# rajgandhi1/threecrate

Measured on AMD Instinct MI355X. Metric: ICP iterations/sec (whole job: k=16 normals + 50-iter point-to-plane ICP per 1M-pt pair; tc_cloud handles, inputs resident in HBM), higher is better.
Workload: dtype f32; 1 GPU; 1000000-pt uniform-random cloud, k=16 normals + 50-iter point-to-plane ICP, independent sigma = 0.0001 noise on source and target, correspondences returned (BASELINE configs[1]; one independent pair per GPU); points=1000000, k=16, parallelism=pairs1, interface=tc_cloud handles (one index build per cloud)

## Files before the change

threecrate_amd/csrc/icp.hip:

```cpp
#include "tc_internal.h"
#include <hip/hip_ext.h>

#include <algorithm>
#include <type_traits>
#include <cmath>
#include <cstring>
#include <cstdlib>
#include <cstdio>

namespace tc {

typedef uint32_t u32x16 __attribute__((ext_vector_type(16)));
struct IcpHeader {
    float q[4], t[3];
    float prev_mse, conv_thr, max_dist;
    uint32_t iterations;
    int32_t done;
    float d_ang, d_t;
    uint32_t d_run;
};
static_assert(offsetof(IcpState, done) == 48 && offsetof(IcpState, max_dist) == 60 && offsetof(IcpState, iterations) == 36 &&
              offsetof(IcpState, prev_mse) == 28 && offsetof(IcpState, conv_thr) == 56, "IcpState header layout");
__device__ __forceinline__ IcpHeader load_header(const IcpState *st) {
    const u32x16 h = *reinterpret_cast<const u32x16 *>(st);
// ... 96 lines not shown
constexpr int kSpanRows = 9;

typedef uint32_t u32x4 __attribute__((ext_vector_type(4)));
typedef uint32_t u32x3 __attribute__((ext_vector_type(3)));

typedef float f32x4 __attribute__((ext_vector_type(4)));
typedef float f32x2 __attribute__((ext_vector_type(2)));

__device__ __forceinline__ float d2_packed(const f32x3 &c, const f32x2 &qxy, float qz) {
    const f32x2 dxy = c.xy - qxy;
    const float dz = c.z - qz;
    const f32x2 sxy = dxy * dxy;
    return (sxy.x + sxy.y) + dz * dz;
}

#ifdef TC_PHASE_STAMPS
#define TC_STAMP(i) do { const unsigned long long t_ = __builtin_amdgcn_s_memtime(); ph[i] += t_ - tl; tl = t_; } while (0)
#define TC_STAMP_ARGS , unsigned long long (&ph)[8], unsigned long long &tl
#define TC_STAMP_PASS , ph, tl
#else
#define TC_STAMP(i) do { } while (0)
#define TC_STAMP_ARGS
#define TC_STAMP_PASS
#endif
template <bool STATS = false, bool T2 = false>
__device__ __forceinline__ void nn_search_pruned(const GridView &gv, float x, float y, float z, float ub2,
                                                 float &best, uint32_t &bestj, bool &refine, float max_dist,
                                                 uint2 (*spans)[kIcpBlock], uint32_t &nsteps, const float *pts12, bool track2, float &low2 TC_STAMP_ARGS
                                                 ) {
    const GridGeom &g = gv.g;
    int cx, cy, cz;
    float out2;
    const float qx = fminf(fmaxf(x, g.minx), g.maxx), qy = fminf(fmaxf(y, g.miny), g.maxy),
                qz = fminf(fmaxf(z, g.minz), g.maxz);
    cx = cell_coord(qx, g.minx, g.inv_h, g.gx);
    cy = cell_coord(qy, g.miny, g.inv_h, g.gy);
    cz = cell_coord(qz, g.minz, g.inv_h, g.gz);
    const float fx = (qx - g.minx) * g.inv_h - (float)cx, fy = (qy - g.miny) * g.inv_h - (float)cy,
                fz = (qz - g.minz) * g.inv_h - (float)cz;
    out2 = outside_d2(x, y, z, qx, qy, qz, g.clamped);
    const float lo_x = fmaxf(fx - 2e-3f, 0.0f) * g.h, hi_x = fmaxf(1.0f - fx - 2e-3f, 0.0f) * g.h;
    const float lo_y = fmaxf(fy - 2e-3f, 0.0f) * g.h, hi_y = fmaxf(1.0f - fy - 2e-3f, 0.0f) * g.h;
    const float lo_z = fmaxf(fz - 2e-3f, 0.0f) * g.h, hi_z = fmaxf(1.0f - fz - 2e-3f, 0.0f) * g.h;
    const float ax2[3] = {lo_x * lo_x, 0.0f, hi_x * hi_x};
    const float ay2[3] = {lo_y * lo_y, 0.0f, hi_y * hi_y};
    const float az2[3] = {lo_z * lo_z, 0.0f, hi_z * hi_z};
// ... 484 lines not shown
#pragma unroll
            for (int w2 = 0; w2 < kIcpBlock / 64; ++w2) sum += red[w2][threadIdx.x];
        }
        partials[(size_t)blockIdx.x * TC_ICP_SUMS_STRIDE + threadIdx.x] = sum;
    }
    if (lane == 0) rlist[blockIdx.x * kWavesPerBlock + w] = wcnt;
    if (blk_times && threadIdx.x == 0) {
        blk_times[2 * blockIdx.x] = t_begin;
        blk_times[2 * blockIdx.x + 1] = __builtin_amdgcn_s_memrealtime();
#ifdef TC_PHASE_STAMPS
        TC_STAMP(6);
        for (int i = 0; i < 8; ++i) blk_times[2 * kMaxPartialBlocks + 8 * blockIdx.x + i] = ph[i];
#endif
    }
}

constexpr int kRefineThreads = 1024;
#ifndef TC_REFINE_LANES
#define TC_REFINE_LANES 32
#endif
constexpr int kRG = TC_REFINE_LANES;
constexpr int kRB = 4;

__device__ __forceinline__ unsigned long long group_min_u64(unsigned long long v) {
#pragma unroll
    for (int o = kRG / 2; o > 0; o >>= 1) {
        const unsigned long long w = __shfl_xor(v, o);
        v = w < v ? w : v;
    }
    return v;
}

__device__ __forceinline__ void shell_cell(int idx, int R, int W, int V, int &ox, int &oy, int &oz) {
    const int nz = 2 * W * W, ny = 2 * W * V;
    if (idx < nz) {
        const int f = idx / (W * W), r = idx - f * W * W;
        oz = f ? R : -R; oy = r / W - R; ox = r - (r / W) * W - R;
    } else if (idx < nz + ny) {
        const int i2 = idx - nz, f = i2 / (W * V), r = i2 - f * W * V;
        oy = f ? R : -R; oz = r / W - (R - 1); ox = r - (r / W) * W - R;
    } else {
        const int i3 = idx - nz - ny, f = i3 / (V * V), r = i3 - f * V * V;
        ox = f ? R : -R; oz = r / V - (R - 1); oy = r - (r / V) * V - (R - 1);
    }
}

// ... 113 lines not shown
                const unsigned long long kc = ka < kb ? ka : kb;
                lk = kc < lk ? kc : lk;
            }
        }
        lim = fminf(lim, __uint_as_float((uint32_t)(lk >> 32)));
        if ((batch & 3u) == 3u) {
            float gl = lim;
#pragma unroll
            for (int o = kRG / 2; o > 0; o >>= 1) gl = fminf(gl, __shfl_xor(gl, o));
            lim = gl;
        }
    }
    return group_min_u64(lk);
}

template <int MODE>
__global__ void __launch_bounds__(kRefineThreads) icp_refine_kernel(
    GridView tgt, const float4 *__restrict__ tgt_nrm, const float4 *__restrict__ src,
    IcpState *__restrict__ st, uint32_t *__restrict__ corr_pos , uint32_t *__restrict__ rlist,
    const double *__restrict__ main_rows, uint32_t n_main_rows, uint32_t seg_stride, double *__restrict__ partial_rows,
    const float4 *__restrict__ src_cov, int dbg) {
    constexpr bool P2PLANE = MODE == 1;
    constexpr int NACC = MODE == 0 ? TC_ICP_SUMS_P2P : TC_ICP_SUMS_P2PLANE;
    const IcpHeader hd = load_header(st);
    const bool dbg_shells = (dbg & 8192) != 0;
    __shared__ float lacc[kRefineThreads / kRG][TC_ICP_SUMS_STRIDE];
    const uint32_t rows_per = (n_main_rows + gridDim.x - 1) / gridDim.x;
    const uint32_t mr0 = min(blockIdx.x * rows_per, n_main_rows), mr1 = min(mr0 + rows_per, n_main_rows);
    constexpr int kFoldBatch = kMaxPartialBlocks / kRefineBlocks;
    double fr[kFoldBatch];
#pragma unroll
    for (int k = 0; k < kFoldBatch; ++k) {
        const double v = main_rows[(size_t)min(mr0 + k, n_main_rows - 1) * TC_ICP_SUMS_STRIDE + (threadIdx.x & (TC_ICP_SUMS_STRIDE - 1))];
        fr[k] = (mr0 + k < mr1) ? v : 0.0;
    }
    constexpr int kSegPerRow = kIcpBlock / 64;
    constexpr int kCntPer = kMaxPartialBlocks * kSegPerRow / kRefineThreads;
    const uint32_t n_segs = n_main_rows * kSegPerRow;
    constexpr uint32_t per = kCntPer;
    uint32_t cnt[kCntPer];
#pragma unroll
    for (int k = 0; k < kCntPer; ++k) {
        const uint32_t b = threadIdx.x * per + k;
        const uint32_t v = rlist[min(b, n_segs - 1)];
        cnt[k] = b < n_segs ? v : 0u;
    }
    if (hd.done) return;
    double folded = 0.0;
#pragma unroll
    for (int k = 0; k < kFoldBatch; ++k) folded += fr[k];
    if (threadIdx.x < TC_ICP_SUMS_STRIDE)
        for (uint32_t r = mr0 + kFoldBatch; r < mr1; ++r) folded += main_rows[(size_t)r * TC_ICP_SUMS_STRIDE + threadIdx.x];
    const GridGeom &g = tgt.g;
    const float q[4] = {hd.q[0], hd.q[1], hd.q[2], hd.q[3]};
    const float max_dist = hd.max_dist;
    __shared__ uint32_t seg_off[kMaxPartialBlocks * kSegPerRow + 1];
    __shared__ uint32_t wave_tot[kRefineThreads / 64];
    {
        uint32_t run = 0;
#pragma unroll
        for (int k = 0; k < kCntPer; ++k) run += cnt[k];
        uint32_t inc = run;
#pragma unroll
        for (int o = 1; o < 64; o <<= 1) {
            const uint32_t v = __shfl_up(inc, o);
            if ((int)(threadIdx.x & 63) >= o) inc += v;
        }
        if ((threadIdx.x & 63) == 63) wave_tot[threadIdx.x >> 6] = inc;
        __syncthreads();
        uint32_t ex = inc - run;
        for (int w2 = 0; w2 < (int)(threadIdx.x >> 6); ++w2) ex += wave_tot[w2];
#pragma unroll
        for (int k = 0; k < kCntPer; ++k) {
            const uint32_t b = threadIdx.x * per + k;
            if (b <= n_segs) seg_off[b] = ex;
            ex += cnt[k];
        }
        if (threadIdx.x == kRefineThreads - 1) seg_off[n_segs] = ex;
        __syncthreads();
    }
    const uint32_t count = seg_off[n_segs];
    const uint4 *__restrict__ entries = refine_entries(rlist);
    if (blockIdx.x == 0 && threadIdx.x == 0) {
        st->refine_total += count;
        st->refine_max = max(st->refine_max, count);
    }
    if ((uint32_t)blockIdx.x >= count) {
        if (threadIdx.x < TC_ICP_SUMS_STRIDE) partial_rows[(size_t)blockIdx.x * TC_ICP_SUMS_STRIDE + threadIdx.x] = folded;
        return;
    }
    const __amdgpu_buffer_rsrc_t pt_rsrc = raw_rsrc(tgt.pts), cs_rsrc = raw_rsrc(tgt.cell_start);
    const int lg = threadIdx.x & (kRG - 1);
    const uint32_t group = (threadIdx.x / kRG) * gridDim.x + blockIdx.x, ngroups = gridDim.x * kRefineThreads / kRG;
    const unsigned long long gmask = (kRG == 64) ? ~0ull : (((1ull << kRG) - 1ull) << ((threadIdx.x & 63) & ~(kRG - 1)));
    float *const acc = lacc[threadIdx.x / kRG];
    for (int k = lg; k < NACC; k += kRG) acc[k] = 0.0f;
    __builtin_amdgcn_fence(__ATOMIC_RELEASE, "wavefront");
    auto locate = [&](uint32_t i) -> size_t {
        uint32_t lo = 0, nleft = n_segs;
        while (nleft > 1) {
            const uint32_t stride = (nleft + kRG - 1) / kRG;
            const bool le = (uint32_t)lg * stride < nleft && seg_off[lo + lg * stride] <= i;
            const uint32_t m = (uint32_t)((__ballot(le) & gmask) >> ((threadIdx.x & 63) & ~(kRG - 1)));
            const uint32_t k = 31u - (uint32_t)__clz((int)m);
            lo += k * stride;
            nleft = min(stride, nleft - k * stride);
        }
        return (size_t)lo * seg_stride + (i - seg_off[lo]);
    };
    uint4 n0 = make_uint4(0, 0, 0, 0), n1 = n0;
    if (group < count) { const size_t a = locate(group); n0 = entries[2 * a]; n1 = entries[2 * a + 1]; }
    for (uint32_t i = group; i < count; i += ngroups) {
        const uint4 e0 = n0, e1 = n1;
        if (i + ngroups < count) { const size_t a = locate(i + ngroups); n0 = entries[2 * a]; n1 = entries[2 * a + 1]; }
        const uint32_t j = e0.w, pj = e1.y;
        const float x = __uint_as_float(e0.x), y = __uint_as_float(e0.y), z = __uint_as_float(e0.z);
        const float qx = fminf(fmaxf(x, g.minx), g.maxx), qy = fminf(fmaxf(y, g.miny), g.maxy),
                    qz = fminf(fmaxf(z, g.minz), g.maxz);
        const int cx = cell_coord(qx, g.minx, g.inv_h, g.gx), cy = cell_coord(qy, g.miny, g.inv_h, g.gy),
                  cz = cell_coord(qz, g.minz, g.inv_h, g.gz);
        const float fx = (qx - g.minx) * g.inv_h - (float)cx, fy = (qy - g.miny) * g.inv_h - (float)cy,
                    fz = (qz - g.minz) * g.inv_h - (float)cz;
        const float out2 = outside_d2(x, y, z, qx, qy, qz, g.clamped);
        unsigned long long bestkey = ~0ull;
        if (pj != 0xFFFFFFFFu) bestkey = ((unsigned long long)e1.x << 32) | pj;
        if (bestkey != ~0ull && !dbg_shells)
            bestkey = refine_ball_scan(tgt, cs_rsrc, pt_rsrc, lg, x, y, z, bestkey, max_dist >= 0.0f ? max_dist * max_dist * 1.0001f : INFINITY);
        else
        for (int R = 2;; ++R) {
            bool touched;
            const unsigned long long lk = (R == 2) ? refine_shell<2>(tgt, cs_rsrc, pt_rsrc, 2, lg, x, y, z, cx, cy, cz, bestkey, touched)
                                                   : refine_shell<0>(tgt, cs_rsrc, pt_rsrc, R, lg, x, y, z, cx, cy, cz, bestkey, touched);
            bestkey = lk < bestkey ? lk : bestkey;
            const bool any_touched = (__ballot(touched) & gmask) != 0ull;
            const bool covers = (cx - R <= 0) && (cx + R >= g.gx - 1) && (cy - R <= 0) && (cy + R >= g.gy - 1) &&
                                (cz - R <= 0) && (cz + R >= g.gz - 1);
            const float big = 1.0e30f;
            const float mf = fmaxf(fminf(fminf(fminf(cx - R >= 1 ? fx : big, cx + R <= g.gx - 2 ? 1.0f - fx : big),
                                               fminf(cy - R >= 1 ? fy : big, cy + R <= g.gy - 2 ? 1.0f - fy : big)),
                                         fminf(cz - R >= 1 ? fz : big, cz + R <= g.gz - 2 ? 1.0f - fz : big)), 0.0f);
            const float bound = ((float)R + mf - 2e-3f) * g.h;
            const float bd = __uint_as_float((uint32_t)(bestkey >> 32));
#ifdef TC_REFINE_STATS
            if (lg == 0 && (covers || !any_touched || (bestkey != ~0ull && bd <= bound * bound + out2) || (max_dist >= 0.0f && bound > max_dist)))
                atomicAdd(const_cast<uint32_t *>(&st->refine_ring_hist[min(R, 7)]), 1u);
#endif
            if (covers || !any_touched) break;
            if (bestkey != ~0ull && bd <= bound * bound + out2) break;
            if (max_dist >= 0.0f && bound > max_dist) break;
            if (bestkey != ~0ull && !(dbg_shells)) {
                bestkey = refine_ball_scan(tgt, cs_rsrc, pt_rsrc, lg, x, y, z, bestkey, max_dist >= 0.0f ? max_dist * max_dist * 1.0001f : INFINITY);
                break;
            }
        }
        if (lg == 0) {
            const float best = __uint_as_float((uint32_t)(bestkey >> 32));
            const uint32_t bestg = (uint32_t)bestkey;
            bool valid = bestkey != ~0ull;
            if (valid && max_dist >= 0.0f) valid = !(sqrtf(best) > max_dist);
            corr_pos[4 * (size_t)j] = valid ? bestg : 0xFFFFFFFFu;
            if (valid) {
                const float4 c = tgt.pts[bestg];
                float a[NACC];
#pragma unroll
                for (int k = 0; k < NACC; ++k) a[k] = acc[k];
                if constexpr (MODE == 2) {
                    float R[9];
                    quat_to_rot(q, R);
                    accumulate_gicp(a, x, y, z, c, best, R, src_cov[2 * (size_t)j], src_cov[2 * (size_t)j + 1], tgt_nrm[2 * (size_t)bestg],
                                    tgt_nrm[2 * (size_t)bestg + 1]);
                } else {
                    float4 n = make_float4(0.f, 0.f, 0.f, 0.f);
                    if (P2PLANE) n = tgt_nrm[bestg];
                    accumulate_pair<P2PLANE, NACC>(g, a, x, y, z, c, n);
                }
#pragma unroll
                for (int k = 0; k < NACC; ++k) acc[k] = a[k];
            }
        }
    }
    __syncthreads();
    if (threadIdx.x < TC_ICP_SUMS_STRIDE) {
        double sum = 0.0;
        if (threadIdx.x < NACC) {
#pragma unroll 8
            for (int g2 = 0; g2 < kRefineThreads / kRG; ++g2) sum += (double)lacc[g2][threadIdx.x];
        }
        partial_rows[(size_t)blockIdx.x * TC_ICP_SUMS_STRIDE + threadIdx.x] = sum + folded;
    }
}

__global__ void __launch_bounds__(256) icp_write_corr_kernel(GridView tgt, const float4 *__restrict__ src, uint32_t ns,
                                                            const uint32_t *__restrict__ corr_pos,
                                                            uint32_t *__restrict__ corr) {
    const uint32_t j = blockIdx.x * blockDim.x + threadIdx.x;
    if (j >= ns) return;
    const uint32_t so = __float_as_uint(src[j].w);
    const uint32_t pj = corr_pos[4 * (size_t)j];
    corr[so] = (pj == 0xFFFFFFFFu) ? 0xFFFFFFFFu : __float_as_uint(tgt.pts[pj].w);
}

__global__ void __launch_bounds__(kIcpBlock) icp_final_mse_kernel(GridView tgt, const float4 *__restrict__ src, uint32_t ns,
                                                                  uint32_t chunk, const IcpState *__restrict__ st,
                                                                  const uint32_t *__restrict__ corr_pos,
                                                                  double *__restrict__ partials) {
    if (st->done) return;
    __shared__ double red[kIcpBlock / 64][TC_ICP_SUMS_STRIDE];
    const float q[4] = {st->q[0], st->q[1], st->q[2], st->q[3]};
    const float t[3] = {st->t[0], st->t[1], st->t[2]};
    double acc[2] = {0.0, 0.0};
    const uint32_t beg = blockIdx.x * chunk, end = min(beg + chunk, ns);
    for (uint32_t j = beg + threadIdx.x; j < end; j += kIcpBlock) {
// ... 170 lines not shown
            const double f = A[r][i] * inv;
            A[r][i] = f;
            for (int c = i + 1; c < 6; ++c) A[r][c] -= f * A[i][c];
            x[r] -= f * x[i];
        }
    }
    for (int i = 5; i >= 0; --i) {
        if (A[i][i] == 0.0) return false;
        double s = x[i];
        for (int c = i + 1; c < 6; ++c) s -= A[i][c] * x[c];
        x[i] = s / A[i][i];
    }
    return true;
}

__device__ __forceinline__ void quat_mul_f(const float a[4], const float b[4], float o[4]) {
    const float w = a[3] * b[3] - a[0] * b[0] - a[1] * b[1] - a[2] * b[2];
    const float i = a[3] * b[0] + a[0] * b[3] + a[1] * b[2] - a[2] * b[1];
    const float j = a[3] * b[1] - a[0] * b[2] + a[1] * b[3] + a[2] * b[0];
    const float k = a[3] * b[2] + a[0] * b[1] - a[1] * b[0] + a[2] * b[3];
    o[0] = i; o[1] = j; o[2] = k; o[3] = w;
}

__device__ void compose(const IcpHeader &hd, IcpState *st, const float dq[4], const float dt[3], const GridGeom &g, double searchers, double pairs, int cert_active) {
    if (cert_active != 0) {
        st->searchers = (uint32_t)fmin(searchers, 4.0e9);
        const bool was_on = hd.d_ang >= 0.0f;
        bool wanted = false;
        float ang = -1.0f, tn = 0.0f;
        if (was_on || searchers > 0.1 * pairs) {
            ang = 2.0f * __builtin_amdgcn_sqrtf(dq[0] * dq[0] + dq[1] * dq[1] + dq[2] * dq[2]) * 1.0001f;
            tn = __builtin_amdgcn_sqrtf(dt[0] * dt[0] + dt[1] * dt[1] + dt[2] * dt[2]) * 1.0001f;
            const float rx_ = fmaxf(fabsf(g.minx), fabsf(g.maxx)), ry_ = fmaxf(fabsf(g.miny), fabsf(g.maxy)), rz_ = fmaxf(fabsf(g.minz), fabsf(g.maxz));
            const float far = __builtin_amdgcn_sqrtf(rx_ * rx_ + ry_ * ry_ + rz_ * rz_) * 1.0001f;
            const float moved = ang * far + tn;
            wanted = ang < 5e-3f && moved < (was_on ? 0.01f : 0.003f) * g.h;
        }
        st->d_ang = wanted ? ang : -1.0f;
        st->d_t = tn;
        st->d_run = (wanted && (cert_active & 1)) ? min(hd.d_run + 1u, 1000000u) : 0u;
    }
    const float cq[4] = {hd.q[0], hd.q[1], hd.q[2], hd.q[3]};
    const float ct[3] = {hd.t[0], hd.t[1], hd.t[2]};
    const float zero[3] = {0.0f, 0.0f, 0.0f};
    float rx, ry, rz;
    isometry_apply(dq, zero, ct[0], ct[1], ct[2], rx, ry, rz);
    float nq[4];
    quat_mul_f(dq, cq, nq);
    st->q[0] = nq[0]; st->q[1] = nq[1]; st->q[2] = nq[2]; st->q[3] = nq[3];
    st->t[0] = dt[0] + rx; st->t[1] = dt[1] + ry; st->t[2] = dt[2] + rz;
}

__device__ void kabsch_rotation(const double Hin[3][3], double R[3][3]) {
    double H[3][3], V[3][3];
    for (int i = 0; i < 3; ++i) for (int j = 0; j < 3; ++j) { H[i][j] = Hin[i][j]; V[i][j] = (i == j) ? 1.0 : 0.0; }
    for (int sweep = 0; sweep < 30; ++sweep) {
        double off = 0.0;
        for (int p = 0; p < 2; ++p) for (int qq = p + 1; qq < 3; ++qq) {
            double alpha = 0, beta = 0, gamma = 0;
            for (int i = 0; i < 3; ++i) { alpha += H[i][p] * H[i][p]; beta += H[i][qq] * H[i][qq]; gamma += H[i][p] * H[i][qq]; }
            if (gamma == 0.0 || fabs(gamma) <= 1e-18 * sqrt(alpha * beta)) continue;
            off = fmax(off, fabs(gamma) / sqrt(alpha * beta));
            const double zeta = (beta - alpha) / (2.0 * gamma);
            const double tt = (zeta >= 0.0 ? 1.0 : -1.0) / (fabs(zeta) + sqrt(1.0 + zeta * zeta));
            const double c = 1.0 / sqrt(1.0 + tt * tt), s = c * tt;
            for (int i = 0; i < 3; ++i) {
                const double hp = H[i][p], hq = H[i][qq];
                H[i][p] = c * hp - s * hq; H[i][qq] = s * hp + c * hq;
                const double vp = V[i][p], vq = V[i][qq];
                V[i][p] = c * vp - s * vq; V[i][qq] = s * vp + c * vq;
            }
        }
        if (off < 1e-15) break;
// ... 33 lines not shown
    }
}

__device__ void rotmat_to_quat(const double m[3][3], float q[4]) {
    const double tr = m[0][0] + m[1][1] + m[2][2];
    double w, i, j, k;
    if (tr > 0.0) {
        const double d = sqrt(tr + 1.0) * 2.0;
        w = 0.25 * d; i = (m[2][1] - m[1][2]) / d; j = (m[0][2] - m[2][0]) / d; k = (m[1][0] - m[0][1]) / d;
    } else if (m[0][0] > m[1][1] && m[0][0] > m[2][2]) {
        const double d = sqrt(1.0 + m[0][0] - m[1][1] - m[2][2]) * 2.0;
        w = (m[2][1] - m[1][2]) / d; i = 0.25 * d; j = (m[0][1] + m[1][0]) / d; k = (m[0][2] + m[2][0]) / d;
    } else if (m[1][1] > m[2][2]) {
        const double d = sqrt(1.0 + m[1][1] - m[0][0] - m[2][2]) * 2.0;
        w = (m[0][2] - m[2][0]) / d; i = (m[0][1] + m[1][0]) / d; j = 0.25 * d; k = (m[1][2] + m[2][1]) / d;
    } else {
        const double d = sqrt(1.0 + m[2][2] - m[0][0] - m[1][1]) * 2.0;
        w = (m[1][0] - m[0][1]) / d; i = (m[0][2] + m[2][0]) / d; j = (m[1][2] + m[2][1]) / d; k = 0.25 * d;
    }
    const double nq = sqrt(w * w + i * i + j * j + k * k);
    q[0] = (float)(i / nq); q[1] = (float)(j / nq); q[2] = (float)(k / nq); q[3] = (float)(w / nq);
}

__device__ void finish_iteration(const IcpHeader &hd, IcpState *st, float mse, uint32_t n) {
    st->iterations = hd.iterations + 1u;
    st->mse = mse;
    st->n_corr = n;
    const float change = fabsf(hd.prev_mse - mse);
    if (change < hd.conv_thr) { st->converged = 1; st->done = 1; return; }
    st->prev_mse = mse;
}

constexpr int kFinalizeThreads = 512;
template <int MODE>
__device__ void finalize_body(const double *__restrict__ partials, uint32_t nblocks, IcpState *__restrict__ st, const GridGeom &g,
                              int do_sum, int do_apply, double (*sm)[TC_ICP_SUMS_STRIDE], const IcpHeader &hd, int cert_active = 0) {
    const bool done = hd.done != 0;
    constexpr bool P2PLANE = MODE != 0;
    if (do_sum) {
        constexpr int G = kFinalizeThreads / 32;
        {
            const int col = threadIdx.x & 31, grp = threadIdx.x >> 5;
            double s0 = 0.0, s1 = 0.0, s2 = 0.0, s3 = 0.0;
            uint32_t b = grp;
            if (nblocks == 256) {
                double v[256 / G];
#pragma unroll
                for (int k = 0; k < 256 / G; ++k) v[k] = partials[(size_t)(grp + G * k) * TC_ICP_SUMS_STRIDE + col];
#pragma unroll
                for (int k = 0; k < 256 / G; k += 4) { s0 += v[k]; s1 += v[k + 1]; s2 += v[k + 2]; s3 += v[k + 3]; }
                b = 256 + grp;
            }
            for (; b + 3 * G < nblocks; b += 4 * G) {
                s0 += partials[(size_t)b * TC_ICP_SUMS_STRIDE + col];
                s1 += partials[(size_t)(b + G) * TC_ICP_SUMS_STRIDE + col];
                s2 += partials[(size_t)(b + 2 * G) * TC_ICP_SUMS_STRIDE + col];
                s3 += partials[(size_t)(b + 3 * G) * TC_ICP_SUMS_STRIDE + col];
            }
            for (; b < nblocks; b += G) s0 += partials[(size_t)b * TC_ICP_SUMS_STRIDE + col];
            sm[grp][col] = (s0 + s1) + (s2 + s3);
        }
        __syncthreads();
        double tot = 0.0;
        if (threadIdx.x < TC_ICP_SUMS_STRIDE) {
#pragma unroll
            for (int gi = 0; gi < G; ++gi) tot += sm[gi][threadIdx.x];
            if (!done) st->sums[threadIdx.x] = tot;
        }
        __syncthreads();
        if (threadIdx.x < TC_ICP_SUMS_STRIDE) sm[0][threadIdx.x] = tot;
        __syncthreads();
    }
    if (!do_apply || threadIdx.x != 0 || done) return;
    const double *S = do_sum ? &sm[0][0] : st->sums;
    if (P2PLANE) {
        const double cnt = S[28];
        if (cnt < 6.0) { st->status = TC_ALGORITHM; st->done = 1; return; }
        double x[6];
        if (!chol6_solve(S, S + 21, x)) {
            __shared__ double sA[6][6], sx[6];
            int o = 0;
#pragma unroll
            for (int r = 0; r < 6; ++r)
#pragma unroll
                for (int c = r; c < 6; ++c) { sA[r][c] = S[o]; sA[c][r] = S[o]; ++o; }
#pragma unroll
            for (int r = 0; r < 6; ++r) sx[r] = S[21 + r];
            if (!lu6_solve(sA, sx)) { st->status = TC_ALGORITHM; st->done = 1; return; }
#pragma unroll
            for (int r = 0; r < 6; ++r) x[r] = sx[r];
        }
        const float hx = (float)x[0] / 2.0f, hy = (float)x[1] / 2.0f, hz = (float)x[2] / 2.0f;
        float sx, cx, sy, cy, sz, cz;
        sincosf(hx, &sx, &cx); sincosf(hy, &sy, &cy); sincosf(hz, &sz, &cz);
        const float qx[4] = {sx, 0.0f, 0.0f, cx};
        const float qy[4] = {0.0f, sy, 0.0f, cy};
        const float qz[4] = {0.0f, 0.0f, sz, cz};
        float zy[4], rot[4];
        quat_mul_f(qz, qy, zy);
        quat_mul_f(zy, qx, rot);
        const float dt[3] = {(float)x[3], (float)x[4], (float)x[5]};
        compose(hd, st, rot, dt, g, S[kSearchersCol], cnt, cert_active);
        finish_iteration(hd, st, (float)(S[27] / cnt), (uint32_t)cnt);
    } else {
        const double cnt = S[16];
        if (cnt < 3.0) { st->status = TC_ALGORITHM; st->done = 1; return; }
        const double ms[3] = {S[0] / cnt, S[1] / cnt, S[2] / cnt}, mq[3] = {S[3] / cnt, S[4] / cnt, S[5] / cnt};
        double H[3][3], R[3][3];
        for (int r = 0; r < 3; ++r) for (int c = 0; c < 3; ++c) H[r][c] = S[6 + 3 * r + c] - cnt * ms[r] * mq[c];
        if (st->kiss) {
            double hn = 0.0;
            for (int r = 0; r < 3; ++r) for (int c = 0; c < 3; ++c) hn += H[r][c] * H[r][c];
            if (sqrt(hn) < 1e-10) { st->status = TC_ALGORITHM; st->done = 1; return; }
        }
        kabsch_rotation(H, R);
        const double cs[3] = {ms[0] + (double)g.cx, ms[1] + (double)g.cy, ms[2] + (double)g.cz};
        const double cq[3] = {mq[0] + (double)g.cx, mq[1] + (double)g.cy, mq[2] + (double)g.cz};
        float dq[4];
        rotmat_to_quat(R, dq);
        float dt[3];
        for (int r = 0; r < 3; ++r) dt[r] = (float)(cq[r] - (R[r][0] * cs[0] + R[r][1] * cs[1] + R[r][2] * cs[2]));
        compose(hd, st, dq, dt, g, S[kSearchersCol], cnt, cert_active);
        double nmse = S[15];
        if (st->kiss) {
            const double d0 = ms[0] - mq[0], d1 = ms[1] - mq[1], d2 = ms[2] - mq[2];
            double rh = 0.0;
            for (int i = 0; i < 3; ++i) for (int j = 0; j < 3; ++j) rh += R[i][j] * H[j][i];
            nmse = S[15] - cnt * (d0 * d0 + d1 * d1 + d2 * d2) + 2.0 * (H[0][0] + H[1][1] + H[2][2]) - 2.0 * rh;
            nmse = fmax(nmse, 0.0);
        }
        finish_iteration(hd, st, (float)(nmse / cnt), (uint32_t)cnt);
    }
}

template <int MODE>
__global__ void __launch_bounds__(kFinalizeThreads) icp_finalize_kernel(const double *__restrict__ partials, uint32_t nblocks,
                                                           IcpState *__restrict__ st, const GridGeom g, int do_sum, int do_apply,
                                                           int32_t *__restrict__ done_out, int cert_active) {
    const IcpHeader hd = load_header(st);
    __shared__ double sm[kFinalizeThreads / 32][TC_ICP_SUMS_STRIDE];
    if (hd.done && !do_sum) { if (done_out && threadIdx.x == 0) __hip_atomic_store(done_out, 1, __ATOMIC_RELAXED, __HIP_MEMORY_SCOPE_SYSTEM); return; }
#ifdef TC_PHASE_STAMPS
    const unsigned long long t0 = __builtin_amdgcn_s_memtime();
    finalize_body<MODE>(partials, nblocks, st, g, do_sum, 0, sm, hd);
    const unsigned long long t1 = __builtin_amdgcn_s_memtime();
    finalize_body<MODE>(partials, nblocks, st, g, 0, do_apply, sm, hd, cert_active | (done_out != nullptr ? 2 : 0));
    const unsigned long long t2 = __builtin_amdgcn_s_memtime();
    if (threadIdx.x == 0) { st->refine_ring_hist[0] += (uint32_t)(t1 - t0); st->refine_ring_hist[1] += (uint32_t)(t2 - t1); }
#else
    finalize_body<MODE>(partials, nblocks, st, g, do_sum, do_apply, sm, hd, cert_active | (done_out != nullptr ? 2 : 0));
#endif
    if (done_out && threadIdx.x == 0)
        __hip_atomic_store(done_out, (hd.done || st->done) ? 1 : (st->d_ang >= 0.0f ? 3 : 2), __ATOMIC_RELAXED, __HIP_MEMORY_SCOPE_SYSTEM);
}

constexpr int kStateWords = (int)(offsetof(IcpState, sums) / sizeof(uint32_t));
static_assert(kStateWords <= 64, "one lane per word");
__device__ __forceinline__ void publish_state(const IcpState *st, IcpState *host_out, uint32_t *lds) {
    if (threadIdx.x == 0) {
        const uint32_t *s = reinterpret_cast<const uint32_t *>(st);
        for (int i = 0; i < kStateWords; ++i) lds[i] = s[i];
    }
    __syncthreads();
    if ((int)threadIdx.x < kStateWords)
        __hip_atomic_store(reinterpret_cast<uint32_t *>(host_out) + threadIdx.x, lds[threadIdx.x], __ATOMIC_RELAXED, __HIP_MEMORY_SCOPE_SYSTEM);
}
__global__ void icp_finish_kernel(IcpState *__restrict__ st, const double *__restrict__ partials, uint32_t nblocks, int p2plane, int from_sums,
                                  IcpState *__restrict__ host_out) {
    __shared__ uint32_t lds[64];
    if (threadIdx.x == 0 && !st->done) {
    st->converged = 0;
    if (p2plane || st->kiss) {
        st->mse = st->prev_mse;
    } else {
        double s = 0.0, c = 0.0;
        if (from_sums) { s = st->sums[0]; c = st->sums[1]; }
// ... 357 lines not shown
        if (tc_status s = ensure(ctx, ctx->dbg_times, 10 * (size_t)kMaxPartialBlocks * sizeof(unsigned long long))) return s;
    if (tc_status s = run_chunked(ctx, job.max_iters, [&](int32_t *done_out) -> tc_status {
            if (enq++ == vor_after() && !vor)
                if (tc_status s = launch_target_nn_bounds(ctx, (*su.tix), su.tv, su.st, &vor)) return s;
            launch_iteration(ctx, su, IcpStep::FullIteration, vor, done_out, ctx->icp_cert);
            return TC_OK;
        })) return s;
    if (mode == 0) {
        ProfScope ps(ctx, "icp_final_mse");
        hipLaunchKernelGGL(icp_final_mse_kernel, dim3(su.l.mse_blocks), dim3(kIcpBlock), 0, st, su.tv, (const float4 *)su.wsrc, (uint32_t)ns,
                           su.l.mse_chunk, su.st, corr_pos, su.partials);
    }
    const IcpState *hs = nullptr;
    if (tc_status s = launch_finish(ctx, su, su.l.mse_blocks, 0, false, &hs)) return s;
    if (res->corr_target) {
        hipLaunchKernelGGL(icp_write_corr_kernel, dim3((unsigned)((ns + 255) / 256)), dim3(256), 0, st, su.tv, su.src, (uint32_t)ns,
                           corr_pos, job.corr_on_device ? res->corr_target : corr);
        if (!job.corr_on_device) TC_HIP_TRY(ctx, hipMemcpyAsync(res->corr_target, corr, ns * sizeof(uint32_t), hipMemcpyDeviceToHost, st));
    }
    TC_HIP_TRY(ctx, hipStreamSynchronize(st));
    TC_HIP_TRY(ctx, hipGetLastError());
    if ((debug_flags() & 1024) && ctx->dbg_times.p) dump_block_schedule(ctx, su.l.nblocks);
    fold_search_stats(ctx, hs);
    if (debug_flags() & 64)
        fprintf(stderr, "[tc] icp: searching lanes at the last evaluation of the certificate's gate %u (d_run %u, wanted %d)\n", hs->searchers, hs->d_run, hs->d_ang >= 0.0f ? 1 : 0);
    if (debug_flags() & 64)
        fprintf(stderr, "[tc] icp: %u iterations, refine queries total %u max %u  exit ring hist %u %u %u %u %u %u %u %u\n", hs->iterations,
                hs->refine_total, hs->refine_max, hs->refine_ring_hist[0], hs->refine_ring_hist[1], hs->refine_ring_hist[2], hs->refine_ring_hist[3],
                hs->refine_ring_hist[4], hs->refine_ring_hist[5], hs->refine_ring_hist[6], hs->refine_ring_hist[7]);
    return fill_result(ctx, hs, job.max_iters,
                       mode == 2 ? "GICP: insufficient correspondences (need >= 6) or ill-conditioned Gauss-Newton system"
                       : mode == 1 ? "Insufficient correspondences for point-to-plane ICP (need >= 6) or ill-conditioned system"
                                   : "Insufficient correspondences found", true, res);
}


__global__ void __launch_bounds__(256) icp_zero_u32_kernel(uint32_t *__restrict__ p, uint32_t n) {
    const uint32_t i = blockIdx.x * blockDim.x + threadIdx.x;
    if (i < n) p[i] = 0u;
}

tc_status icp_run_sharded(tc_context *ctx, tc_comm *comm, int shard_mode, const IcpJob &job, tc_icp_result *res) {
    const int mode = job.mode;
    const size_t ns = job.ns, max_iters = job.max_iters;
    const int W = comm ? comm->nranks : 1, rank = comm ? comm->rank : 0;
    IcpSetup su;
// ... 148 lines not shown
```

Measured before the change: 18040 it/s.

## Shorten ICP refine and finalize kernel tails with earlier loads and wave-local solve

```diff
diff --git a/threecrate_amd/csrc/icp.hip b/threecrate_amd/csrc/icp.hip
--- a/threecrate_amd/csrc/icp.hip
+++ b/threecrate_amd/csrc/icp.hip
@@ -142,6 +142,30 @@
 #define TC_STAMP(i) do { } while (0)
 #define TC_STAMP_ARGS
 #define TC_STAMP_PASS
+#endif
+#ifdef TC_PHASE_STAMPS
+constexpr int kTailSlots = 10;
+__device__ unsigned long long g_tail_stamps[3][kTailSlots + 2];
+#define TC_TAIL_ARGS , unsigned long long (&tt_)[kTailSlots]
+#define TC_TAIL_PASS , tt_
+#define TC_TAIL_BEGIN() unsigned long long tt_[kTailSlots] = {0, 0, 0, 0, 0, 0, 0, 0, 0, 0}; const unsigned long long tr0_ = __builtin_amdgcn_s_memrealtime(); tt_[0] = __builtin_amdgcn_s_memtime()
+#define TC_TAIL(i) do { tt_[i] = __builtin_amdgcn_s_memtime(); } while (0)
+#define TC_TAIL_SMEM(i) do { asm volatile("s_waitcnt lgkmcnt(0)" ::: "memory"); TC_TAIL(i); } while (0)
+#define TC_TAIL_VMEM(i) do { asm volatile("s_waitcnt vmcnt(0)" ::: "memory"); TC_TAIL(i); } while (0)
+#define TC_TAIL_AFTER(i, value) do { asm volatile("" :: "v"(value)); TC_TAIL(i); } while (0)
+#define TC_TAIL_FLUSH(kind) do { \
+        for (int i_ = 1; i_ < kTailSlots; ++i_) if (tt_[i_]) atomicAdd(&g_tail_stamps[kind][i_], tt_[i_] - tt_[0]); \
+        atomicAdd(&g_tail_stamps[kind][kTailSlots], 1ull); \
+        atomicAdd(&g_tail_stamps[kind][kTailSlots + 1], __builtin_amdgcn_s_memrealtime() - tr0_); } while (0)
+#else
+#define TC_TAIL_ARGS
+#define TC_TAIL_PASS
+#define TC_TAIL_BEGIN() do { } while (0)
+#define TC_TAIL(i) do { } while (0)
+#define TC_TAIL_SMEM(i) do { } while (0)
+#define TC_TAIL_VMEM(i) do { } while (0)
+#define TC_TAIL_AFTER(i, value) do { } while (0)
+#define TC_TAIL_FLUSH(kind) do { } while (0)
 #endif
 template <bool STATS = false, bool T2 = false>
 __device__ __forceinline__ void nn_search_pruned(const GridView &gv, float x, float y, float z, float ub2,
@@ -672,6 +696,20 @@
 constexpr int kRG = TC_REFINE_LANES;
 constexpr int kRB = 4;
 
+template <int CTRL, int ROW_MASK>
+__device__ __forceinline__ uint32_t dpp_or_zero(uint32_t v) {
+    return (uint32_t)__builtin_amdgcn_update_dpp(0, (int)v, CTRL, ROW_MASK, 0xF, false);
+}
+__device__ __forceinline__ uint32_t wave_scan_u32(uint32_t v) {
+    v += dpp_or_zero<0x111, 0xF>(v);
+    v += dpp_or_zero<0x112, 0xF>(v);
+    v += dpp_or_zero<0x114, 0xF>(v);
+    v += dpp_or_zero<0x118, 0xF>(v);
+    v += dpp_or_zero<0x142, 0xA>(v);
+    v += dpp_or_zero<0x143, 0xC>(v);
+    return v;
+}
+
 __device__ __forceinline__ unsigned long long group_min_u64(unsigned long long v) {
 #pragma unroll
     for (int o = kRG / 2; o > 0; o >>= 1) {
@@ -831,7 +869,7 @@
     const float4 *__restrict__ src_cov, int dbg) {
     constexpr bool P2PLANE = MODE == 1;
     constexpr int NACC = MODE == 0 ? TC_ICP_SUMS_P2P : TC_ICP_SUMS_P2PLANE;
-    const IcpHeader hd = load_header(st);
+    TC_TAIL_BEGIN();
     const bool dbg_shells = (dbg & 8192) != 0;
     __shared__ float lacc[kRefineThreads / kRG][TC_ICP_SUMS_STRIDE];
     const uint32_t rows_per = (n_main_rows + gridDim.x - 1) / gridDim.x;
@@ -840,7 +878,8 @@
     double fr[kFoldBatch];
 #pragma unroll
     for (int k = 0; k < kFoldBatch; ++k) {
-        const double v = main_rows[(size_t)min(mr0 + k, n_main_rows - 1) * TC_ICP_SUMS_STRIDE + (threadIdx.x & (TC_ICP_SUMS_STRIDE - 1))];
+        const double v = __hip_atomic_load(&main_rows[(size_t)min(mr0 + k, n_main_rows - 1) * TC_ICP_SUMS_STRIDE + (threadIdx.x & (TC_ICP_SUMS_STRIDE - 1))],
+                                           __ATOMIC_RELAXED, __HIP_MEMORY_SCOPE_WAVEFRONT);
         fr[k] = (mr0 + k < mr1) ? v : 0.0;
     }
     constexpr int kSegPerRow = kIcpBlock / 64;
@@ -854,7 +893,11 @@
         const uint32_t v = rlist[min(b, n_segs - 1)];
         cnt[k] = b < n_segs ? v : 0u;
     }
+    asm volatile("" ::: "memory");
+    const IcpHeader hd = load_header(st);
+    TC_TAIL_SMEM(1);
     if (hd.done) return;
+    TC_TAIL_VMEM(2);
     double folded = 0.0;
 #pragma unroll
     for (int k = 0; k < kFoldBatch; ++k) folded += fr[k];
@@ -865,20 +908,34 @@
     const float max_dist = hd.max_dist;
     __shared__ uint32_t seg_off[kMaxPartialBlocks * kSegPerRow + 1];
     __shared__ uint32_t wave_tot[kRefineThreads / 64];
+    uint32_t count = 0;
     {
         uint32_t run = 0;
 #pragma unroll
         for (int k = 0; k < kCntPer; ++k) run += cnt[k];
-        uint32_t inc = run;
-#pragma unroll
-        for (int o = 1; o < 64; o <<= 1) {
-            const uint32_t v = __shfl_up(inc, o);
-            if ((int)(threadIdx.x & 63) >= o) inc += v;
-        }
+        const uint32_t inc = wave_scan_u32(run);
         if ((threadIdx.x & 63) == 63) wave_tot[threadIdx.x >> 6] = inc;
         __syncthreads();
         uint32_t ex = inc - run;
-        for (int w2 = 0; w2 < (int)(threadIdx.x >> 6); ++w2) ex += wave_tot[w2];
+#pragma unroll
+        for (int w2 = 0; w2 < kRefineThreads / 64; ++w2) {
+            const uint32_t wt = wave_tot[w2];
+            count += wt;
+            if (w2 < (int)(threadIdx.x >> 6)) ex += wt;
+        }
+        TC_TAIL_AFTER(3, count);
+        if (blockIdx.x == 0 && threadIdx.x == 0) {
+            st->refine_total += count;
+            st->refine_max = max(st->refine_max, count);
+        }
+        if ((uint32_t)blockIdx.x >= count) {
+            TC_TAIL_AFTER(4, folded);
+            if (threadIdx.x < TC_ICP_SUMS_STRIDE) partial_rows[(size_t)blockIdx.x * TC_ICP_SUMS_STRIDE + threadIdx.x] = folded;
+#ifdef TC_PHASE_STAMPS
+            if (blockIdx.x == gridDim.x - 1 && threadIdx.x == 0) { TC_TAIL(5); TC_TAIL_FLUSH(1); }
+#endif
+            return;
+        }
 #pragma unroll
         for (int k = 0; k < kCntPer; ++k) {
             const uint32_t b = threadIdx.x * per + k;
@@ -888,16 +945,8 @@
         if (threadIdx.x == kRefineThreads - 1) seg_off[n_segs] = ex;
         __syncthreads();
     }
-    const uint32_t count = seg_off[n_segs];
     const uint4 *__restrict__ entries = refine_entries(rlist);
-    if (blockIdx.x == 0 && threadIdx.x == 0) {
-        st->refine_total += count;
-        st->refine_max = max(st->refine_max, count);
-    }
-    if ((uint32_t)blockIdx.x >= count) {
-        if (threadIdx.x < TC_ICP_SUMS_STRIDE) partial_rows[(size_t)blockIdx.x * TC_ICP_SUMS_STRIDE + threadIdx.x] = folded;
-        return;
-    }
+    TC_TAIL(4);
     const __amdgpu_buffer_rsrc_t pt_rsrc = raw_rsrc(tgt.pts), cs_rsrc = raw_rsrc(tgt.cell_start);
     const int lg = threadIdx.x & (kRG - 1);
     const uint32_t group = (threadIdx.x / kRG) * gridDim.x + blockIdx.x, ngroups = gridDim.x * kRefineThreads / kRG;
@@ -921,6 +970,9 @@
     if (group < count) { const size_t a = locate(group); n0 = entries[2 * a]; n1 = entries[2 * a + 1]; }
     for (uint32_t i = group; i < count; i += ngroups) {
         const uint4 e0 = n0, e1 = n1;
+#ifdef TC_PHASE_STAMPS
+        if (i == group) { asm volatile("" :: "v"(e0.x), "v"(e1.y)); TC_TAIL(5); }
+#endif
         if (i + ngroups < count) { const size_t a = locate(i + ngroups); n0 = entries[2 * a]; n1 = entries[2 * a + 1]; }
         const uint32_t j = e0.w, pj = e1.y;
         const float x = __uint_as_float(e0.x), y = __uint_as_float(e0.y), z = __uint_as_float(e0.z);
@@ -962,6 +1014,9 @@
                 break;
             }
         }
+#ifdef TC_PHASE_STAMPS
+        if (i == group) { asm volatile("" :: "v"((uint32_t)bestkey)); TC_TAIL(6); }
+#endif
         if (lg == 0) {
             const float best = __uint_as_float((uint32_t)(bestkey >> 32));
             const uint32_t bestg = (uint32_t)bestkey;
@@ -988,6 +1043,7 @@
             }
         }
     }
+    TC_TAIL(7);
     __syncthreads();
     if (threadIdx.x < TC_ICP_SUMS_STRIDE) {
         double sum = 0.0;
@@ -997,6 +1053,9 @@
         }
         partial_rows[(size_t)blockIdx.x * TC_ICP_SUMS_STRIDE + threadIdx.x] = sum + folded;
     }
+#ifdef TC_PHASE_STAMPS
+    if (blockIdx.x == 0 && threadIdx.x == 0) { TC_TAIL(8); TC_TAIL_FLUSH(2); }
+#endif
 }
 
 __global__ void __launch_bounds__(256) icp_write_corr_kernel(GridView tgt, const float4 *__restrict__ src, uint32_t ns,
@@ -1213,7 +1272,8 @@
     o[0] = i; o[1] = j; o[2] = k; o[3] = w;
 }
 
-__device__ void compose(const IcpHeader &hd, IcpState *st, const float dq[4], const float dt[3], const GridGeom &g, double searchers, double pairs, int cert_active) {
+__device__ float compose(const IcpHeader &hd, IcpState *st, const float dq[4], const float dt[3], const GridGeom &g, double searchers, double pairs, int cert_active) {
+    float d_ang_now = hd.d_ang;
     if (cert_active != 0) {
         st->searchers = (uint32_t)fmin(searchers, 4.0e9);
         const bool was_on = hd.d_ang >= 0.0f;
@@ -1227,7 +1287,8 @@
             const float moved = ang * far + tn;
             wanted = ang < 5e-3f && moved < (was_on ? 0.01f : 0.003f) * g.h;
         }
-        st->d_ang = wanted ? ang : -1.0f;
+        d_ang_now = wanted ? ang : -1.0f;
+        st->d_ang = d_ang_now;
         st->d_t = tn;
         st->d_run = (wanted && (cert_active & 1)) ? min(hd.d_run + 1u, 1000000u) : 0u;
     }
@@ -1240,6 +1301,7 @@
     quat_mul_f(dq, cq, nq);
     st->q[0] = nq[0]; st->q[1] = nq[1]; st->q[2] = nq[2]; st->q[3] = nq[3];
     st->t[0] = dt[0] + rx; st->t[1] = dt[1] + ry; st->t[2] = dt[2] + rz;
+    return d_ang_now;
 }
 
 __device__ void kabsch_rotation(const double Hin[3][3], double R[3][3]) {
@@ -1319,33 +1381,44 @@
     q[0] = (float)(i / nq); q[1] = (float)(j / nq); q[2] = (float)(k / nq); q[3] = (float)(w / nq);
 }
 
-__device__ void finish_iteration(const IcpHeader &hd, IcpState *st, float mse, uint32_t n) {
+__device__ bool finish_iteration(const IcpHeader &hd, IcpState *st, float mse, uint32_t n) {
     st->iterations = hd.iterations + 1u;
     st->mse = mse;
     st->n_corr = n;
     const float change = fabsf(hd.prev_mse - mse);
-    if (change < hd.conv_thr) { st->converged = 1; st->done = 1; return; }
+    if (change < hd.conv_thr) { st->converged = 1; st->done = 1; return true; }
     st->prev_mse = mse;
+    return false;
 }
 
 constexpr int kFinalizeThreads = 512;
+constexpr int kFinalizeGroups = kFinalizeThreads / 32;
+constexpr int kFinalizeBatch = 256 / kFinalizeGroups;
+struct TailOut { int done; float d_ang; };
+__device__ __forceinline__ float lane_value(float v, int lane) {
+    return __builtin_bit_cast(float, __builtin_amdgcn_readlane(__builtin_bit_cast(int, v), lane));
+}
+__device__ __forceinline__ void wave_lds_fence() {
+    __builtin_amdgcn_fence(__ATOMIC_RELEASE, "wavefront");
+    __builtin_amdgcn_wave_barrier();
+    __builtin_amdgcn_fence(__ATOMIC_ACQUIRE, "wavefront");
+}
 template <int MODE>
-__device__ void finalize_body(const double *__restrict__ partials, uint32_t nblocks, IcpState *__restrict__ st, const GridGeom &g,
-                              int do_sum, int do_apply, double (*sm)[TC_ICP_SUMS_STRIDE], const IcpHeader &hd, int cert_active = 0) {
+__device__ __forceinline__ TailOut finalize_body(const double *__restrict__ partials, uint32_t nblocks, IcpState *__restrict__ st, const GridGeom &g,
+                                                 int do_sum, int do_apply, double (*sm)[TC_ICP_SUMS_STRIDE], const IcpHeader &hd,
+                                                 const double (&v)[kFinalizeBatch], int cert_active TC_TAIL_ARGS) {
     const bool done = hd.done != 0;
+    const TailOut unchanged = {hd.done, hd.d_ang}, failed = {1, hd.d_ang};
     constexpr bool P2PLANE = MODE != 0;
+    constexpr int G = kFinalizeGroups;
     if (do_sum) {
-        constexpr int G = kFinalizeThreads / 32;
         {
             const int col = threadIdx.x & 31, grp = threadIdx.x >> 5;
             double s0 = 0.0, s1 = 0.0, s2 = 0.0, s3 = 0.0;
             uint32_t b = grp;
             if (nblocks == 256) {
-                double v[256 / G];
-#pragma unroll
-                for (int k = 0; k < 256 / G; ++k) v[k] = partials[(size_t)(grp + G * k) * TC_ICP_SUMS_STRIDE + col];
-#pragma unroll
-                for (int k = 0; k < 256 / G; k += 4) { s0 += v[k]; s1 += v[k + 1]; s2 += v[k + 2]; s3 += v[k + 3]; }
+#pragma unroll
+                for (int k = 0; k < kFinalizeBatch; k += 4) { s0 += v[k]; s1 += v[k + 1]; s2 += v[k + 2]; s3 += v[k + 3]; }
                 b = 256 + grp;
             }
             for (; b + 3 * G < nblocks; b += 4 * G) {
@@ -1358,38 +1431,53 @@
             sm[grp][col] = (s0 + s1) + (s2 + s3);
         }
         __syncthreads();
+    }
+    if (threadIdx.x >= 64) return unchanged;
+    if (threadIdx.x < TC_ICP_SUMS_STRIDE) {
         double tot = 0.0;
-        if (threadIdx.x < TC_ICP_SUMS_STRIDE) {
+        if (do_sum) {
 #pragma unroll
             for (int gi = 0; gi < G; ++gi) tot += sm[gi][threadIdx.x];
             if (!done) st->sums[threadIdx.x] = tot;
-        }
-        __syncthreads();
-        if (threadIdx.x < TC_ICP_SUMS_STRIDE) sm[0][threadIdx.x] = tot;
-        __syncthreads();
-    }
-    if (!do_apply || threadIdx.x != 0 || done) return;
-    const double *S = do_sum ? &sm[0][0] : st->sums;
+        } else if (do_apply && !done) {
+            tot = st->sums[threadIdx.x];
+        }
+        sm[0][threadIdx.x] = tot;
+    }
+    if (!do_apply || done) return unchanged;
+    wave_lds_fence();
+    const double *S = &sm[0][0];
+    TC_TAIL_AFTER(3, S[28]);
     if (P2PLANE) {
         const double cnt = S[28];
-        if (cnt < 6.0) { st->status = TC_ALGORITHM; st->done = 1; return; }
+        if (cnt < 6.0) { if (threadIdx.x == 0) { st->status = TC_ALGORITHM; st->done = 1; } return failed; }
         double x[6];
         if (!chol6_solve(S, S + 21, x)) {
-            __shared__ double sA[6][6], sx[6];
-            int o = 0;
-#pragma unroll
-            for (int r = 0; r < 6; ++r)
-#pragma unroll
-                for (int c = r; c < 6; ++c) { sA[r][c] = S[o]; sA[c][r] = S[o]; ++o; }
-#pragma unroll
-            for (int r = 0; r < 6; ++r) sx[r] = S[21 + r];
-            if (!lu6_solve(sA, sx)) { st->status = TC_ALGORITHM; st->done = 1; return; }
-#pragma unroll
-            for (int r = 0; r < 6; ++r) x[r] = sx[r];
+            __shared__ double sA[6][6], lx[6];
+            __shared__ int lu_ok;
+            if (threadIdx.x == 0) {
+                int o = 0;
+#pragma unroll
+                for (int r = 0; r < 6; ++r)
+#pragma unroll
+                    for (int c = r; c < 6; ++c) { sA[r][c] = S[o]; sA[c][r] = S[o]; ++o; }
+#pragma unroll
+                for (int r = 0; r < 6; ++r) lx[r] = S[21 + r];
+                lu_ok = lu6_solve(sA, lx) ? 1 : 0;
+            }
+            wave_lds_fence();
+            if (!lu_ok) { if (threadIdx.x == 0) { st->status = TC_ALGORITHM; st->done = 1; } return failed; }
+#pragma unroll
+            for (int r = 0; r < 6; ++r) x[r] = lx[r];
         }
         const float hx = (float)x[0] / 2.0f, hy = (float)x[1] / 2.0f, hz = (float)x[2] / 2.0f;
-        float sx, cx, sy, cy, sz, cz;
-        sincosf(hx, &sx, &cx); sincosf(hy, &sy, &cy); sincosf(hz, &sz, &cz);
+        TC_TAIL_AFTER(4, hx + hy + hz);
+        const float ha = threadIdx.x == 1 ? hy : threadIdx.x == 2 ? hz : hx;
+        float sa, ca;
+        sincosf(ha, &sa, &ca);
+        const float sx = lane_value(sa, 0), cx = lane_value(ca, 0), sy = lane_value(sa, 1), cy = lane_value(ca, 1),
+                    sz = lane_value(sa, 2), cz = lane_value(ca, 2);
+        if (threadIdx.x != 0) return unchanged;
         const float qx[4] = {sx, 0.0f, 0.0f, cx};
         const float qy[4] = {0.0f, sy, 0.0f, cy};
         const float qz[4] = {0.0f, 0.0f, sz, cz};
@@ -1397,18 +1485,23 @@
         quat_mul_f(qz, qy, zy);
         quat_mul_f(zy, qx, rot);
         const float dt[3] = {(float)x[3], (float)x[4], (float)x[5]};
-        compose(hd, st, rot, dt, g, S[kSearchersCol], cnt, cert_active);
-        finish_iteration(hd, st, (float)(S[27] / cnt), (uint32_t)cnt);
+        TailOut out;
+        out.d_ang = compose(hd, st, rot, dt, g, S[kSearchersCol], cnt, cert_active);
+        TC_TAIL_AFTER(5, out.d_ang);
+        out.done = finish_iteration(hd, st, (float)(S[27] / cnt), (uint32_t)cnt) ? 1 : 0;
+        TC_TAIL(6);
+        return out;
     } else {
+        if (threadIdx.x != 0) return unchanged;
         const double cnt = S[16];
-        if (cnt < 3.0) { st->status = TC_ALGORITHM; st->done = 1; return; }
+        if (cnt < 3.0) { st->status = TC_ALGORITHM; st->done = 1; return failed; }
         const double ms[3] = {S[0] / cnt, S[1] / cnt, S[2] / cnt}, mq[3] = {S[3] / cnt, S[4] / cnt, S[5] / cnt};
         double H[3][3], R[3][3];
         for (int r = 0; r < 3; ++r) for (int c = 0; c < 3; ++c) H[r][c] = S[6 + 3 * r + c] - cnt * ms[r] * mq[c];
         if (st->kiss) {
             double hn = 0.0;
             for (int r = 0; r < 3; ++r) for (int c = 0; c < 3; ++c) hn += H[r][c] * H[r][c];
-            if (sqrt(hn) < 1e-10) { st->status = TC_ALGORITHM; st->done = 1; return; }
+            if (sqrt(hn) < 1e-10) { st->status = TC_ALGORITHM; st->done = 1; return failed; }
         }
         kabsch_rotation(H, R);
         const double cs[3] = {ms[0] + (double)g.cx, ms[1] + (double)g.cy, ms[2] + (double)g.cz};
@@ -1417,7 +1510,8 @@
         rotmat_to_quat(R, dq);
         float dt[3];
         for (int r = 0; r < 3; ++r) dt[r] = (float)(cq[r] - (R[r][0] * cs[0] + R[r][1] * cs[1] + R[r][2] * cs[2]));
-        compose(hd, st, dq, dt, g, S[kSearchersCol], cnt, cert_active);
+        TailOut out;
+        out.d_ang = compose(hd, st, dq, dt, g, S[kSearchersCol], cnt, cert_active);
         double nmse = S[15];
         if (st->kiss) {
             const double d0 = ms[0] - mq[0], d1 = ms[1] - mq[1], d2 = ms[2] - mq[2];
@@ -1426,7 +1520,8 @@
             nmse = S[15] - cnt * (d0 * d0 + d1 * d1 + d2 * d2) + 2.0 * (H[0][0] + H[1][1] + H[2][2]) - 2.0 * rh;
             nmse = fmax(nmse, 0.0);
         }
-        finish_iteration(hd, st, (float)(nmse / cnt), (uint32_t)cnt);
+        out.done = finish_iteration(hd, st, (float)(nmse / cnt), (uint32_t)cnt) ? 1 : 0;
+        return out;
     }
 }
 
@@ -1434,21 +1529,27 @@
 __global__ void __launch_bounds__(kFinalizeThreads) icp_finalize_kernel(const double *__restrict__ partials, uint32_t nblocks,
                                                            IcpState *__restrict__ st, const GridGeom g, int do_sum, int do_apply,
                                                            int32_t *__restrict__ done_out, int cert_active) {
+    TC_TAIL_BEGIN();
+    __shared__ double sm[kFinalizeGroups][TC_ICP_SUMS_STRIDE];
+    double v[kFinalizeBatch];
+#pragma unroll
+    for (int k = 0; k < kFinalizeBatch; ++k) v[k] = 0.0;
+    if (do_sum && nblocks == 256) {
+        const int col = threadIdx.x & 31, grp = threadIdx.x >> 5;
+#pragma unroll
+        for (int k = 0; k < kFinalizeBatch; ++k) v[k] = partials[(size_t)(grp + kFinalizeGroups * k) * TC_ICP_SUMS_STRIDE + col];
+    }
+    asm volatile("" ::: "memory");
     const IcpHeader hd = load_header(st);
-    __shared__ double sm[kFinalizeThreads / 32][TC_ICP_SUMS_STRIDE];
+    TC_TAIL_SMEM(1);
     if (hd.done && !do_sum) { if (done_out && threadIdx.x == 0) __hip_atomic_store(done_out, 1, __ATOMIC_RELAXED, __HIP_MEMORY_SCOPE_SYSTEM); return; }
+    TC_TAIL_VMEM(2);
+    const TailOut out = finalize_body<MODE>(partials, nblocks, st, g, do_sum, do_apply, sm, hd, v, cert_active | (done_out != nullptr ? 2 : 0) TC_TAIL_PASS);
+    if (done_out && threadIdx.x == 0)
+        __hip_atomic_store(done_out, (hd.done || out.done) ? 1 : (out.d_ang >= 0.0f ? 3 : 2), __ATOMIC_RELAXED, __HIP_MEMORY_SCOPE_SYSTEM);
 #ifdef TC_PHASE_STAMPS
-    const unsigned long long t0 = __builtin_amdgcn_s_memtime();
-    finalize_body<MODE>(partials, nblocks, st, g, do_sum, 0, sm, hd);
-    const unsigned long long t1 = __builtin_amdgcn_s_memtime();
-    finalize_body<MODE>(partials, nblocks, st, g, 0, do_apply, sm, hd, cert_active | (done_out != nullptr ? 2 : 0));
-    const unsigned long long t2 = __builtin_amdgcn_s_memtime();
-    if (threadIdx.x == 0) { st->refine_ring_hist[0] += (uint32_t)(t1 - t0); st->refine_ring_hist[1] += (uint32_t)(t2 - t1); }
-#else
-    finalize_body<MODE>(partials, nblocks, st, g, do_sum, do_apply, sm, hd, cert_active | (done_out != nullptr ? 2 : 0));
+    if (threadIdx.x == 0) { TC_TAIL(7); TC_TAIL_FLUSH(0); }
 #endif
-    if (done_out && threadIdx.x == 0)
-        __hip_atomic_store(done_out, (hd.done || st->done) ? 1 : (st->d_ang >= 0.0f ? 3 : 2), __ATOMIC_RELAXED, __HIP_MEMORY_SCOPE_SYSTEM);
 }
 
 constexpr int kStateWords = (int)(offsetof(IcpState, sums) / sizeof(uint32_t));
@@ -1852,6 +1953,21 @@
     TC_HIP_TRY(ctx, hipGetLastError());
     if ((debug_flags() & 1024) && ctx->dbg_times.p) dump_block_schedule(ctx, su.l.nblocks);
     fold_search_stats(ctx, hs);
+#ifdef TC_PHASE_STAMPS
+    if (debug_flags() & 64) {
+        unsigned long long h[3][kTailSlots + 2], zero[3][kTailSlots + 2] = {};
+        (void)hipMemcpyFromSymbol(h, HIP_SYMBOL(g_tail_stamps), sizeof h);
+        (void)hipMemcpyToSymbol(HIP_SYMBOL(g_tail_stamps), zero, sizeof zero);
+        static const char *const kind[3] = {"icp_finalize", "icp_refine last block, no query", "icp_refine block 0, with queries"};
+        for (int k = 0; k < 3; ++k) {
+            const double n = (double)std::max<unsigned long long>(h[k][kTailSlots], 1);
+            fprintf(stderr, "[tc] tail stamps: %s: %llu launches, %.3f us each by s_memrealtime; mean s_memtime ticks from entry:", kind[k], h[k][kTailSlots],
+                    h[k][kTailSlots + 1] / n * 0.01);
+            for (int i = 1; i < kTailSlots; ++i) fprintf(stderr, " [%d] %.0f", i, h[k][i] / n);
+            fprintf(stderr, "\n");
+        }
+    }
+#endif
     if (debug_flags() & 64)
         fprintf(stderr, "[tc] icp: searching lanes at the last evaluation of the certificate's gate %u (d_run %u, wanted %d)\n", hs->searchers, hs->d_run, hs->d_ang >= 0.0f ? 1 : 0);
     if (debug_flags() & 64)
```

New measurement: 18330 it/s (median of 6 runs). 1.6% higher.
